# parlance/ctcdecode

Hardware: AMD Instinct MI355X
Metric: utterances/sec at B=256 T=1000 V=29 beam=100 (higher is better)
Workload: dtype f32; 1 GPU; BASELINE.json configs[1]: CTC prefix beam search, no LM, log-softmax of N(0,1) logits; HBM-resident tensors (input in HBM, the four result tensors left in HBM: `e2e`, with --full, is the host-to-host call); utterances_per_gpu=256, frames=1000, vocab=29, beam_width=100, cutoff_top_n=29, global_batch=256, ranks=1, devices_visible=1, parallelism=single GPU, threads_per_workgroup=default

## Files before the change

ctcdecode_amd/csrc/beam_core.h:

```cpp
#pragma once
#include <stddef.h>
#include <stdint.h>

#include "exact_math.h"
#include "exact_math_f64.h"
#include "lm_tables.h"
#include "stl_emul.h"
#if defined(CTC_ASSUME_CHECKED)
#include <cstdio>
#include <cstdlib>
#endif

#define CTC_RARE(x) __builtin_expect(!!(x), 0)
#if !defined(CTC_SPEC_UP)
#define CTC_SPEC_UP 1.5f
#endif
#if !defined(CTC_SPEC_DN)
#define CTC_SPEC_DN 0.7f
#endif
#if !defined(CTC_SPEC_OVER_SHIFT)
#define CTC_SPEC_OVER_SHIFT 2
#endif
#define CTC_USUAL(x) __builtin_expect(!!(x), 1)

namespace ctcbeam {

struct alignas(16) Int4v { int x, y, z, w; };

struct PoolNode {
  int32_t parent;
  float lpc;
  uint32_t cht;
  CTC_HD int ch() const { const uint32_t c = cht & 0xFFFFu; return c == 0xFFFFu ? -1 : (int)c; }
  CTC_HD static uint32_t pack(int ch, int tstep) { return ((uint32_t)ch & 0xFFFFu) | ((uint32_t)tstep << 16); }
};

struct EkWide { uint64_t k; uint32_t slot, pad; };
template <bool HUGE> struct EkOps;
template <> struct EkOps<false> {
  using E = uint64_t; using Pos = uint16_t;
  CTC_HD static E make(uint64_t key48v, int slot) { return (key48v << 16) | (uint64_t)slot; }
  CTC_HD static uint64_t key(const E &e) { return e >> 16; }
  CTC_HD static int slot(const E &e) { return (int)(e & 0xFFFFu); }
};
template <> struct EkOps<true> {
  using E = EkWide; using Pos = uint32_t;
  CTC_HD static E make(uint64_t key48v, int slot) { E e; e.k = key48v; e.slot = (uint32_t)slot; e.pad = 0; return e; }
  CTC_HD static uint64_t key(const E &e) { return e.k; }
  CTC_HD static int slot(const E &e) { return (int)e.slot; }
};

enum : uint32_t { T_SELF = 0, T_CHILD = 1, T_REVIVED = 2, T_HOLE = 3 };
enum : int { ST_OK = 0, ST_POOL_OVERFLOW = 1, ST_BAD_CONFIG = 2 };

constexpr int kMaxBeam = 16383;
constexpr int kMaxVocab = 65534;
constexpr int kIntMax = 0x7fffffff;

CTC_HD uint32_t ord_f32(float f) {
  const uint32_t u = ctcmath::f32_to_bits(f + 0.0f);
  return u ^ ((uint32_t)((int32_t)u >> 31) | 0x80000000u);
}
CTC_HD uint32_t ord_f32_raw(float f) {
  const uint32_t u = ctcmath::f32_to_bits(f);
  return u ^ ((uint32_t)((int32_t)u >> 31) | 0x80000000u);
}
CTC_HD float unord_f32(uint32_t k) {
  return ctcmath::bits_to_f32((k & 0x80000000u) ? (k ^ 0x80000000u) : ~k);
}
CTC_HD uint32_t mk_info(int ch, uint32_t type, int entry) {
  return ((uint32_t)(0xFFFF - (ch + 1)) << 16) | (type << 14) | (uint32_t)entry;
}
CTC_HD uint32_t info_type(uint32_t info) { return (info >> 14) & 3u; }
CTC_HD int info_entry(uint32_t info) { return (int)(info & 0x3FFFu); }
CTC_HD int info_ch(uint32_t info) { return 0xFFFF - (int)(info >> 16) - 1; }
CTC_HD uint64_t key48(uint32_t skey, uint32_t info) { return ((uint64_t)skey << 16) | (info >> 16); }
constexpr uint32_t kHoleInfo = T_HOLE << 14;

struct Beam {
  int *node, *par, *ch, *dep, *lcp, *via, *viaanc, *viach;
  int *up;
  float *bprev, *nbprev, *score, *lpc;
  int *lmst, *lmcl;
  int *acc_lo, *acc_hi;
  int *dn, *dmlo, *dmhi, *dfc;
  int *spc_lo, *spc_hi;
  int *spst, *spcl;
};
constexpr int kBeamArrays = 13, kBeamArraysLm = 12;

struct Dims {
  int K;
  int V;
  int Vc_max;
  int use_rank_table;
  int lm;
  CTC_HD int S_max() const { return K * (2 + Vc_max); }
};

enum {
  VAR_STATUS = 0, VAR_CUT, VAR_TAUC,
  VAR_INTO,
  VAR_FB0 = 4, VAR_FB1, VAR_FB2, VAR_FB3,
  VAR_TAU = 8, VAR_G, VAR_E,
  VAR_DANGER,
  VAR_PAR0 = 12,
  P_NPIN = 0, P_LCOUNT, P_NMAXKEY, P_NMINKEY, P_NCAND, P_SIZE = 8,
  VAR_SPEC = VAR_PAR0 + 2 * P_SIZE, SP_THR = 0, SP_WLOG, SP_ANCHOR, SP_PRED, SP_BEST, SP_MARGIN, SP_GAP, SP_ROWMAX,
  VAR_ROWMAX = VAR_SPEC + SP_ROWMAX,
  VAR_QSTAT = VAR_SPEC + 9,
  VAR_LMMISS = VAR_SPEC + 8,
  VAR_LMQ = VAR_SPEC + 10,
  VAR_HOTN = VAR_SPEC + 4,
  VAR_COUNT = VAR_SPEC + 12
};
constexpr int kBins = 1024;
constexpr int kBinsLog = 10;
constexpr int kListCap = 128;
constexpr int kSmallK = 128, kSmallV = 32;
constexpr int kMidK = 112, kMidVc = 40, kMidV = 10240;
constexpr int kWideK = 500, kWideV = 29;
CTC_HD constexpr Dims fixed_layout_dims(bool lm = false) { return Dims{kSmallK, kSmallV, kSmallV, 1, lm ? 1 : 0}; }
CTC_HD bool fits_fixed_layout(const Dims &d) { return d.K <= kSmallK && d.V <= kSmallV && d.Vc_max <= kSmallV; }
CTC_HD constexpr Dims mid_layout_dims() { return Dims{kMidK, kMidV, kMidVc, 1, 0}; }
CTC_HD bool fits_mid_layout(const Dims &d) { return d.K <= kMidK && d.V <= kMidV && d.Vc_max <= kMidVc && d.use_rank_table && !d.lm; }
CTC_HD constexpr Dims wide_layout_dims() { return Dims{kWideK, kWideV, kWideV, 0, 0}; }
CTC_HD bool fits_wide_layout(const Dims &d) { return d.K <= kWideK && d.V <= kWideV && d.Vc_max <= kWideV && !d.use_rank_table && !d.lm; }
constexpr int kHotCap = 256;
#if !defined(CTC_SERIAL_CUT)
#define CTC_SERIAL_CUT 12
#endif
constexpr int kSerialCut = CTC_SERIAL_CUT;
constexpr int kExpress = 32;
enum Event { EV_FRAMES, EV_CANDIDATES, EV_EXACT, EV_INTERNAL, EV_PINNED, EV_LPC_UPDATE, EV_DEAD_PARENT, EV_REVIVE_CAND, EV_REVIVED, EV_WALK,
             EV_WALK_HOPS, EV_FAST_SELECT, EV_SINGLE_KEY, EV_BUCKET_KEYS, EV_SPEC_OK, EV_SPEC_UNDER, EV_SPEC_OVER, EV_SPEC_OTHER, EV_SPEC_HOT,
             EV_SLOW_BELOW, EV_SLOW_CROWDED, EV_SLOW_SINGLE, EV_SLOW_ROUNDS, EV_TIE_FRAMES, EV_TIE_KEYS, EV_TIE_BIG, EV_WIDE_LIST, EV_HOT_LIST, EV_COUNT };

struct Work {
  Beam cur, nxt, beam0;
  size_t beam_blk;
  size_t beam_blk_far;
  size_t blk_via, blk_lm;
  int *e, *anc, *ostart, *cstart, *pinr, *revr;
  int *ancbuf, *acntbuf;
  uint32_t *hit;
  float *b_new, *nb_new, *sc_new, *rev_lpc;
  int *cch;
  float *clp;
  float *clpbuf;
  int16_t *rank_of;
  uint32_t *skey, *sinfo, *pos;
  int *surv;
  uint64_t *ek;
  uint16_t *lr;
  uint32_t *wpre;
  int *bins;
  int *hotge;
  int *lcpst;
  uint32_t *list;
  int *lslot;
  uint32_t *bitmap;
  int *fin, *sstack;
  int stage_skey;
  int *apos;
  int *vars;
};

template <class P>
CTC_HD P *carve_ptr(char *&p, size_t count) {
  P *r = reinterpret_cast<P *>(p);
  p += ((count * sizeof(P) + 15) / 16) * 16;
  return r;
}

template <int BIG, bool FARREP = false>
CTC_HD size_t carve(Work &w, char *base, char *far, const Dims &d, size_t *far_bytes) {
  char *p = base;
  char *q = far;
  constexpr bool deep = BIG >= 2;
  constexpr bool huge = BIG >= 3;
  const size_t K = (size_t)d.K, S = (size_t)d.S_max();
  const size_t Kr = ((K * 4 + 15) / 16) * 16;
  Beam *bs[2] = {&w.cur, &w.nxt};
  constexpr bool lm_far = BIG != 0;
  const size_t n_lm = d.lm ? (size_t)kBeamArraysLm : 0;
  w.beam_blk = (size_t)(kBeamArrays - (deep ? 3 : 0) + (lm_far ? 0 : n_lm)) * Kr;
  w.beam_blk_far = ((deep ? 3 : 0) + (lm_far ? n_lm : 0)) * Kr;
  w.blk_via = deep ? w.beam_blk_far : w.beam_blk;
  w.blk_lm = lm_far ? w.beam_blk_far : w.beam_blk;
  for (int i = 0; i < 2; ++i) {
    Beam &b = *bs[i];
    char *f = q + (size_t)i * w.beam_blk_far;
    b.node = carve_ptr<int>(p, K); b.par = carve_ptr<int>(p, K); b.ch = carve_ptr<int>(p, K);
    b.dep = carve_ptr<int>(p, K); b.lcp = carve_ptr<int>(p, K);
    char *&pv3 = deep ? f : p;
    b.via = carve_ptr<int>(pv3, K); b.viaanc = carve_ptr<int>(pv3, K); b.viach = carve_ptr<int>(pv3, K);
    b.up = carve_ptr<int>(p, K);
    b.bprev = carve_ptr<float>(p, K); b.nbprev = carve_ptr<float>(p, K); b.score = carve_ptr<float>(p, K);
    b.lpc = carve_ptr<float>(p, K);
    const size_t Kl = d.lm ? K : 0;
    char *&pl = lm_far ? f : p;
    b.lmst = carve_ptr<int>(pl, Kl); b.lmcl = carve_ptr<int>(pl, Kl); b.acc_lo = carve_ptr<int>(pl, Kl); b.acc_hi = carve_ptr<int>(pl, Kl);
    b.dn = carve_ptr<int>(pl, Kl); b.dmlo = carve_ptr<int>(pl, Kl); b.dmhi = carve_ptr<int>(pl, Kl); b.dfc = carve_ptr<int>(pl, Kl);
    b.spc_lo = carve_ptr<int>(pl, Kl); b.spc_hi = carve_ptr<int>(pl, Kl); b.spst = carve_ptr<int>(pl, Kl); b.spcl = carve_ptr<int>(pl, Kl);
  }
  q += 2 * w.beam_blk_far;
  w.beam0 = w.cur;
  w.e = carve_ptr<int>(p, K); w.ancbuf = carve_ptr<int>(p, 2 * K); w.acntbuf = carve_ptr<int>(p, 2 * K); w.anc = w.ancbuf;
  w.ostart = carve_ptr<int>(p, K);
  w.cstart = carve_ptr<int>(p, K);
  w.pinr = carve_ptr<int>(deep ? q : p, K);
  w.revr = carve_ptr<int>(deep ? q : p, K); w.hit = carve_ptr<uint32_t>(p, 2 * K);
  w.b_new = carve_ptr<float>(p, K); w.nb_new = carve_ptr<float>(p, K); w.sc_new = carve_ptr<float>(p, K);
  w.rev_lpc = carve_ptr<float>(deep ? q : p, K);
  w.cch = carve_ptr<int>(p, (size_t)d.Vc_max);
  w.clpbuf = carve_ptr<float>(p, 2 * (size_t)d.Vc_max); w.clp = w.clpbuf;
  w.rank_of = carve_ptr<int16_t>(p, d.use_rank_table ? (size_t)d.V : 0);
  w.skey = carve_ptr<uint32_t>(deep ? q : p, S);
  w.surv = carve_ptr<int>(p, 3 * K + 4);
  const size_t lcap = (d.K <= kSmallK && d.Vc_max <= kMidVc) ? (size_t)kHotCap + 64 : (size_t)kListCap + 4;
  w.bins = carve_ptr<int>(p, kBins + kBins / 16 + 4); w.list = carve_ptr<uint32_t>(p, lcap);
  w.lslot = carve_ptr<int>(p, lcap);
  w.hotge = carve_ptr<int>(p, lcap > (size_t)kListCap + 4 ? (size_t)kHotCap : 0);
#if defined(CTC_EXP_LCP_TABLE)
  w.lcpst = carve_ptr<int>(p, (lcap > (size_t)kListCap + 4 && !d.lm) ? (size_t)7 * kSmallK : 0);
#else
  w.lcpst = nullptr;
#endif
  w.bitmap = carve_ptr<uint32_t>(huge ? q : p, 2 * ((S + 63) / 64 + 17));
  w.wpre = huge ? carve_ptr<uint32_t>(q, (S + 63) / 64 + 2) : reinterpret_cast<uint32_t *>(w.bins);
  w.fin = carve_ptr<int>(BIG ? q : p, d.lm ? 2 * K : K);
  w.apos = carve_ptr<int>(BIG ? q : p, K);
  w.sstack = carve_ptr<int>(p, 3 * (2 * 32 + 2));
  w.vars = carve_ptr<int>(p, VAR_COUNT);
  w.sinfo = carve_ptr<uint32_t>(p, BIG ? K : S);
  w.pos = carve_ptr<uint32_t>(BIG ? q : p, K + 2);
  char *&rr = (BIG || FARREP) ? q : p;
  w.ek = carve_ptr<uint64_t>(rr, huge ? 2 * S : S); w.lr = carve_ptr<uint16_t>(rr, (2 * S + 2) * (huge ? 2 : 1));
  w.stage_skey = deep ? 0 : 1;
  if (far_bytes) *far_bytes = (size_t)(q - far);
  return (size_t)(p - base);
}

struct StreamState {
  int *hdr;
  int *arrays;
  int finish;
};
enum { SH_FRAMES = 0, SH_N, SH_POOL, SH_WLOG, SH_MAXKEY, SH_DANGER, SH_MINKEY,
       SH_SP_PRED, SH_SP_GAP, SH_SP_MARGIN,
       SH_WORDS = 12 };
constexpr int kStateArrays = 14;
constexpr int kStateArraysLm = kStateArrays + kBeamArraysLm;
CTC_HD int state_arrays(int lm) { return lm ? kStateArraysLm : kStateArrays; }

struct StepIn {
  int t;
  int Vc;
  int blank_rank;
  int identity;
  float blank_prob;
};


CTC_HD int div_p2(int v, int d) { return v >> __builtin_ctz((unsigned)d); }
CTC_HD int ceil_div_p2(int v, int d) { return div_p2(v + d - 1, d); }

CTC_HD double ctc_log_f64(double v) {
  return ctcmath::log_f64(v, ctcmath::tables64());
}

CTC_HD int ceil_log2_u32(uint32_t v) {
  return v <= 1u ? 0 : 32 - __builtin_clz(v - 1u);
}
CTC_HD int ceil_log2_u64(uint64_t v) {
  return v <= 1 ? 0 : 64 - __builtin_clzll(v - 1);
}

struct OutRefs {
  int32_t *tok, *ts;
  float *score;
  int32_t *len;
  int32_t *n_results;
  int K, T_stride;
  int32_t *c_hdr, *c_ent;
  uint32_t *c_rag;
  unsigned *c_count;
  unsigned c_cap;
  int32_t *m_hdr, *m_ent, *m_done;
  uint32_t *m_rag;
  unsigned m_cap;
};
enum : int { ST_COMPACT_OVERFLOW = 3, ST_INPUT_TIMEOUT = 4,
             ST_NEED_HOST = 5,
             ST_CB_DANGER = 6 };

struct SlotCtx {
  const Beam *pb;
  int n, Vnb, brank;
  uint64_t vmagic;
};

template <class X>
struct FullSyncView {
  X &x;
  CTC_HD int tid() const { return x.tid(); }
  CTC_HD int nt() const { return x.nt(); }
  CTC_HD void sync() { x.sync_full(); }
  CTC_HD int uni(int v) const { return x.uni(v); }
  CTC_HD void block_scan_u32(uint32_t mine, uint32_t *base_out, uint32_t *total_out) { x.block_scan_u32(mine, base_out, total_out); }
  CTC_HD int lanes() const { return x.lanes(); }
  CTC_HD auto ballot(bool p) const { return x.ballot(p); }
  template <class M> CTC_HD int count(M m) const { return x.count(m); }
  template <class M> CTC_HD int count_below(M m) const { return x.count_below(m); }
  CTC_HD uint32_t first_lane(uint32_t v) const { return x.first_lane(v); }
};

#if defined(CTC_ASSUME_CHECKED)
#define CTC_ASSUME(c) do { if (!(c)) { std::fprintf(stderr, "beam_core.h:%d: assumption violated: %s\n", __LINE__, #c); std::abort(); } } while (0)
#elif defined(__clang__)
#define CTC_ASSUME(c) __builtin_assume(c)
#else
#define CTC_ASSUME(c) do { if (!(c)) __builtin_unreachable(); } while (0)
#endif

template <class X, bool IDENT, int SMALLV = 0, bool LM = false, bool LAZY = false, bool FARREP = LAZY, bool HUGE = false, bool WORDLM = false, bool CB = false>
struct Decoder {
  using EO = EkOps<HUGE>;
  using Ek = typename EO::E;
  using LrT = typename EO::Pos;
  static constexpr int kClsK = SMALLV == 2 ? kMidK : kSmallK, kClsVc = SMALLV == 2 ? kMidVc : kSmallV, kClsSlots = kClsK * (2 + kClsVc);
  CTC_HD Ek *ekp() const { return reinterpret_cast<Ek *>(w.ek); }
  CTC_HD LrT *lrp() const { return reinterpret_cast<LrT *>(w.lr); }
  X &x;
  Work &w;
  const Dims d;
  const int blank;
  PoolNode *pool;
  int *pool_up;
  int *pool_thi;
  bool long_t = false;
  const int pool_cap;
  const uint64_t *tbl;
  const ctclm::LmView *lm;

  CTC_HD Decoder(X &x_, Work &w_, const Dims &d_, int blank_, PoolNode *pool_, int *pool_up_, int pool_cap_, const uint64_t *tbl_,
                 const ctclm::LmView *lm_ = nullptr)
      : x(x_), w(w_), d(d_), blank(blank_), pool(pool_), pool_up(pool_up_), pool_thi(pool_up_ + pool_cap_), pool_cap(pool_cap_), tbl(tbl_), lm(lm_) {
    if (LM) {
      const ctclm::DictNode root = lm->dict[0];
      root_lo = (int)root.mask_lo; root_hi = (int)root.mask_hi; root_fc = (int)root.first_child;
      lm_char_v = lm->char_based != 0; lm_wide_v = lm->dict_wide != 0; lm_space = lm->space_id;
      lm_alpha = lm->alpha; lm_beta = lm->beta;
      lm_dict = lm->dict;
    }
  }
  CTC_HD int node_tstep(const PoolNode &pn, int id) const { return (int)(pn.cht >> 16) | (CTC_RARE(long_t) ? pool_thi[id] << 16 : 0); }
  CTC_HD void set_node_time(int id, int ch, int tstep, float lpc) const {
    pool[id].lpc = lpc;
    pool[id].cht = PoolNode::pack(ch, tstep);
    if (CTC_RARE(long_t)) pool_thi[id] = tstep >> 16;
  }

  CTC_HD float lse(float a, float b) const { return ctcmath::lse(a, b, tbl); }

  static constexpr bool kRankEpoch = SMALLV == 2 && !IDENT && X::kRankEpoch;
  CTC_HD static int16_t rank_tag(int t, int r) { return (int16_t)(uint16_t)((((uint32_t)t & 1023u) << 6) | (uint32_t)r); }
  static constexpr bool kTailZero = IDENT && SMALLV && !LAZY && X::kZeroKeyTail;
  CTC_HD void zero_key_tail(int from) {
    if (!kTailZero) return;
    for (int i = from + x.tid(); i < kClsSlots; i += x.nt()) w.skey[i] = 0u;
  }

  static constexpr bool kSpec = SMALLV && (!LM || (X::kSpecLm && !CB)) && !LAZY && X::kSpecSelect;
#if defined(CTC_EXP_HOT_PRELIST)
  static constexpr bool kHotPre = LAZY && !LM && !SMALLV && !HUGE;
#else
  static constexpr bool kHotPre = false;
#endif
  struct HotPre { uint32_t thr; int cap; uint32_t *key; int *slot; };
  uint32_t st_gap = 0;
  uint32_t hot_anchor = 0;
  static constexpr bool kA1Overlap = kSpec && X::kA1Overlap;
  static constexpr bool kLcpTable = kSpec && X::kLcpTable;
  static constexpr bool kParentRec = !SMALLV && !LM && X::kParentRec && !kHotPre;
  static constexpr bool kLmOverlap = LM && WORDLM && SMALLV && !CB && !LAZY && X::kLmOverlap;
  static constexpr uint32_t kLmSpaceDeferred = 0x80000000u;
  CTC_HD void spec_learn(bool selected, uint32_t tau, int hot, int K) const {
    int *sp = w.vars + VAR_SPEC;
    const int pred = sp[SP_PRED];
    const float best = ctcmath::bits_to_f32((uint32_t)sp[SP_BEST]);
    float margin = ctcmath::bits_to_f32((uint32_t)sp[SP_MARGIN]);
    const uint32_t anchor = (uint32_t)sp[SP_ANCHOR];
    int wl = 32;
    float cut = 0.f;
    if (selected) {
      if (pred) {
        if (hot < K) margin = margin < 32.f ? margin * CTC_SPEC_UP : margin;
        else if (hot > K + (K >> CTC_SPEC_OVER_SHIFT) + 3) margin = margin > 0.001f ? margin * CTC_SPEC_DN : margin;
      }
      cut = (best - unord_f32(tau)) + margin;
      const uint32_t kgap = anchor > tau ? anchor - tau : 0u;
      wl = (kgap ? 32 - __builtin_clz(kgap) : 0) + 1;
      wl = wl < kBinsLog ? kBinsLog : (wl > 32 ? 32 : wl);
    }
    sp[SP_MARGIN] = (int)ctcmath::f32_to_bits(margin); sp[SP_GAP] = (int)ctcmath::f32_to_bits(cut);
    sp[SP_PRED] = selected ? 1 : 0; sp[SP_WLOG] = wl;
  }
  CTC_HD void spec_predict(int t) const {
    int *sp = w.vars + VAR_SPEC;
    const int pred = sp[SP_PRED];
    const float rowmax = ctcmath::bits_to_f32((uint32_t)sp[SP_ROWMAX]), cut = ctcmath::bits_to_f32((uint32_t)sp[SP_GAP]);
    const uint32_t mk = (uint32_t)pvars(t - 1)[P_NMAXKEY];
    const float best = unord_f32(mk) + rowmax;
    uint32_t k = ord_f32(best - cut);
    k = k ? k : 1u;
    k = pred ? k : 0xFFFFFFFFu;
    sp[SP_THR] = (int)k; sp[SP_BEST] = (int)ctcmath::f32_to_bits(best); sp[SP_ANCHOR] = (int)mk;
  }

  int st_n = 1, st_pool = 1, st_wlog = 32;
  uint32_t st_maxkey = 0;
  uint32_t st_minkey = 0;
  int root_lo = 0, root_hi = 0, root_fc = 0;
  bool lm_char_v = false, lm_wide_v = false;
  CTC_HD bool lm_char_() const { return !WORDLM && lm_char_v; }
  CTC_HD bool lm_wide_() const { return !WORDLM && lm_wide_v; }
  int lm_space = -1;
  double lm_alpha = 0.0, lm_beta = 0.0;
  const ctclm::DictNode *lm_dict = nullptr;
  static constexpr bool lm_cb = LM && CB;
  CTC_HD int *fin_cur() const { return w.fin + (lm_cb ? st_par * d.K : 0); }
  CTC_HD int *fin_nxt() const { return w.fin + (lm_cb ? (st_par ^ 1) * d.K : 0); }
  static constexpr int kLmqFilter = 256;
  CTC_HD static uint32_t *lmq_filter() {
#if defined(__HIP_DEVICE_COMPILE__)
    __shared__ uint32_t f[kLmqFilter];
#else
    static thread_local uint32_t f[kLmqFilter];
#endif
    return f;
  }
  CTC_HD void lmq_filter_clear() {
    if constexpr (lm_cb)
      for (int i = x.tid(); i < kLmqFilter; i += x.nt()) lmq_filter()[i] = 0u;
  }
  CTC_HD bool lmq_first(uint32_t state, uint32_t word) const {
    if constexpr (lm_cb) {
      if (lm->cb != 1) return true;
      const uint32_t h = ctclm::ng_hash(state, word);
      const uint32_t fp = ((state * 0x85EBCA77u) ^ (word * 0xC2B2AE3Du) ^ (h >> 8)) | 1u;
      uint32_t *e = lmq_filter() + (h & (kLmqFilter - 1));
      if (*e == fp) return false;
      *e = fp;
    }
    return true;
  }
  CTC_HD double lm_cond_(uint32_t *st, int *cl, uint32_t word, bool *missed = nullptr) const {
    const uint32_t st0 = *st;
    const int cl0 = *cl;
    const double v = ctclm::lm_cond(*lm, st, cl, word);
    if (CTC_RARE(lm_cb)) {
      if (v != v) {
        w.vars[VAR_LMMISS] = 1;
        if (lmq_first(st0, word)) {
          unsigned i = x.global_add(lm->cb_count, 1u);
          if (lm->cb_ring) i &= lm->cb_cap - 1;
          if (i < lm->cb_cap) lm->cb_miss[i] = ctclm::MissEntry{st0, word, (uint32_t)x.item(), 1u};
          x.atomic_add(&w.vars[VAR_LMQ], 1);
        }
// ... 542 lines not shown
      uint32_t *wl = reinterpret_cast<uint32_t *>(w.nxt.node);
      const int hot_n = kHotPre ? x.uni(w.vars[VAR_HOTN]) : 0;
      const bool from_hot = kHotPre && !wide && hp.thr != 0xFFFFFFFFu && hp.thr <= b32 && hot_n <= hp.cap;
      if (tid == 0 && from_hot) x.count(EV_HOT_LIST, 1);
      rank_bucket_ext(S, pv, b32, bspan, true, K - fb[1], fb[1], fb[3], wide ? wl : w.list, wide ? reinterpret_cast<int *>(wl + wcap + 4) : w.lslot,
                  from_hot ? &hp : nullptr, hot_n);
      return true;
    }
#else
    (void)hp;
    if (CTC_USUAL(fb[0] >= 0 && fb[3] <= kListCap && (wd.shift != 0 || fb[0] == kBins - 1))) {
      const uint32_t b32 = wd.lo + ((uint32_t)fb[0] << wd.shift);
      const uint32_t bspan = fb[0] == kBins - 1 ? 0xFFFFFFFFu - b32 : (1u << wd.shift) - 1u;
      if (tid == 0) { x.count(EV_FAST_SELECT, 1); x.count(EV_BUCKET_KEYS, fb[3]); if (fb[3] == 1) x.count(EV_SINGLE_KEY, 1); }
      if (kHotPre) {
        const int hot_n = x.uni(w.vars[VAR_HOTN]);
        const bool from_hot = hp.thr != 0xFFFFFFFFu && hp.thr <= b32 && hot_n <= hp.cap;
        if (tid == 0 && from_hot) x.count(EV_HOT_LIST, 1);
        rank_bucket_ext(S, pv, b32, bspan, true, K - fb[1], fb[1], fb[3], w.list, w.lslot, from_hot ? &hp : nullptr, hot_n);
      } else {
        rank_bucket(S, pv, b32, bspan, true, K - fb[1], fb[1], fb[3]);
      }
      return true;
    }
#endif
    uint64_t lo = wd.lo, hi = (uint64_t)1 << 32;
    int shift = wd.shift;
    int need = K, gbase = 0;
    bool first = true;
    for (;;) {
      const int bstar = fb[0], above = fb[1], total = fb[2], inb = fb[3];
      uint64_t blo = 0, bhi = 0;
      bool again = true;
      if (tid == 0) x.count(EV_SLOW_ROUNDS, 1);
      if (bstar < 0) {
        if (tid == 0) x.count(EV_SLOW_BELOW, 1);
        gbase += total; need -= total; hi = lo; lo = 1;
      } else {
        blo = lo + ((uint64_t)bstar << shift);
        bhi = (bstar == kBins - 1) ? hi : blo + ((uint64_t)1 << shift);
        if (bhi > hi) bhi = hi;
        if (shift == 0 && bstar < kBins - 1) {
          if (tid == 0) x.count(EV_SLOW_SINGLE, 1);
          if (tid == 0) { w.vars[VAR_TAU] = (int)(uint32_t)blo; w.vars[VAR_G] = gbase + above; w.vars[VAR_E] = inb; }
          x.sync();
          return false;
        }
        if (inb <= kListCap) again = false;
        else { if (tid == 0) x.count(EV_SLOW_CROWDED, 1); gbase += above; need -= above; lo = blo; hi = bhi; }
      }
      if (!again) {
        rank_bucket<true>(S, pv, (uint32_t)blo, (uint32_t)(bhi - blo - 1), first, need - above, gbase + above, inb);
        return first;
      }
      first = false;
      for (int i = tid; i < kBins; i += nt) w.bins[i] = 0;
      x.sync();
      const uint64_t width = hi - lo;
      shift = width <= (uint64_t)kBins ? 0 : ceil_log2_u64(width) - kBinsLog;
      const uint32_t lo32 = (uint32_t)lo, span = (uint32_t)(hi - lo - 1);
      for (int s0 = tid; s0 < S; s0 += 4 * nt) {
        uint32_t kk[4];
        for (int u = 0; u < 4; ++u) kk[u] = s0 + u * nt < S ? w.skey[s0 + u * nt] : 0u;
        for (int u = 0; u < 4; ++u) {
          const uint32_t k = kk[u], dk = k - lo32;
          if (k >= lo32 && dk <= span) {
            const uint32_t bk = dk >> shift;
            const int bb = bk < (uint32_t)(kBins - 1) ? (int)bk : kBins - 1;
            x.atomic_add(&w.bins[bb], 1);
          }
        }
      }
      x.sync();
      x.find_bucket(w.bins, need, &w.vars[VAR_FB0]);
      x.uni4(&w.vars[VAR_FB0], fb);
    }
  }

  CTC_HD bool resolve_by_character(int S, uint32_t tau, int m, int E, int *pv, const SlotCtx *lz = nullptr) {
    const int tid = x.tid(), nt = x.nt();
    if (E > kListCap) return false;
    if (tid == 0) { pv[P_LCOUNT] = 0; w.vars[VAR_CUT] = 0; }
    x.sync();
    for (int s = tid; s < S; s += nt)
      if (w.skey[s] == tau) w.list[x.atomic_add(&pv[P_LCOUNT], 1)] = ((LAZY ? info_of_slot(*lz, s) : w.sinfo[s]) >> 16) + 1u;
    x.sync();
    for (int q = tid; q < E; q += nt) {
      const uint32_t mine = w.list[q];
      int g = 0, e = 0;
      for (int r = 0; r < E; ++r) {
        const uint32_t o = w.list[r];
        g += o > mine;
        e += o == mine;
      }
      if (g < m && m <= g + e) { w.vars[VAR_TAUC] = (int)(mine - 1u); w.vars[VAR_CUT] = (g + e == m) ? 1 : 2; }
    }
    x.sync();
    return x.uni(w.vars[VAR_CUT]) == 1;
  }

  CTC_HD void build_lcp_table(const Beam &b, int n, int lane) const {
    int *st = w.lcpst;
    const int i0 = lane, i1 = lane + 64;
    int v0 = i0 < n ? b.lcp[i0] : kIntMax, v1 = i1 < n ? b.lcp[i1] : kIntMax;
    st[i0] = v0; st[i1] = v1;
    x.wave_lds_fence();
#if defined(__clang__)
#pragma unroll
#endif
    for (int l = 1; l <= 6; ++l) {
      const int h = 1 << (l - 1);
      const int *p = st + (l - 1) * kSmallK;
      const int a = p[i0 + h];
      const int c = i1 + h < kSmallK ? p[i1 + h] : kIntMax;
      v0 = a < v0 ? a : v0; v1 = c < v1 ? c : v1;
      st[l * kSmallK + i0] = v0; st[l * kSmallK + i1] = v1;
      x.wave_lds_fence();
    }
  }
  CTC_HD int lca_depth_tbl(int ja, int jb) const {
    const int lo = ja < jb ? ja : jb, hi = ja < jb ? jb : ja;
    const int len = hi - lo;
    const int l = 31 - __builtin_clz((unsigned)(len > 0 ? len : 1));
    const int *p = w.lcpst + l * kSmallK;
    const int same = w.cur.dep[ja];
    const int a = p[lo + 1 < kSmallK ? lo + 1 : kSmallK - 1], c = p[hi - (1 << l) + 1];
    const int m = a < c ? a : c;
    return len == 0 ? same : m;
  }
  CTC_HD int lca_depth(int ja, int jb) const {
    const Beam &b = w.cur;
    if (ja == jb) return b.dep[ja];
    const int lo = ja < jb ? ja : jb, hi = ja < jb ? jb : ja;
    int m = kIntMax;
    for (int i = lo + 1; i <= hi; i += 8) {
      const int i1 = i + 1 < hi ? i + 1 : hi, i2 = i + 2 < hi ? i + 2 : hi, i3 = i + 3 < hi ? i + 3 : hi;
      const int i4 = i + 4 < hi ? i + 4 : hi, i5 = i + 5 < hi ? i + 5 : hi, i6 = i + 6 < hi ? i + 6 : hi, i7 = i + 7 < hi ? i + 7 : hi;
      const int l0 = b.lcp[i], l1 = b.lcp[i1], l2 = b.lcp[i2], l3 = b.lcp[i3];
      const int l4 = b.lcp[i4], l5 = b.lcp[i5], l6 = b.lcp[i6], l7 = b.lcp[i7];
      const int m01 = l0 < l1 ? l0 : l1, m23 = l2 < l3 ? l2 : l3, m45 = l4 < l5 ? l4 : l5, m67 = l6 < l7 ? l6 : l7;
      const int ma = m01 < m23 ? m01 : m23, mb = m45 < m67 ? m45 : m67;
      const int mm = ma < mb ? ma : mb;
      m = mm < m ? mm : m;
    }
    return m;
  }

  template <class XX>
  CTC_HD int hoare_round(XX &xx, Ek *v, int first, int last, LrT *Lp, LrT *Rp) {
    if (FARREP) return stlemu::hoare_round_parallel<true>(xx, v, first, last, [](const Ek &e) { return EO::key(e); }, Lp, Rp, &w.vars[VAR_CUT]);
    return stlemu::hoare_round_parallel_chunks(xx, v, first, last, [](const Ek &e) { return EO::key(e); }, Lp, Rp, &w.vars[VAR_CUT]);
  }

  template <class XX>
  CTC_HD bool replay_nth_element(XX &fx, int N, int K) {
    const int tid = x.tid(), nt = x.nt();
    Ek *v = ekp();
    LrT *lr = lrp();
    auto before = [](const Ek &a, const Ek &c) { return EO::key(a) > EO::key(c); };
    int first = 0, last = N, depth = 2 * stlemu::floor_lg(N);
    if (!FARREP) {
      while (last - first > kSerialCut && depth > 0) {
        --depth;
        const int cut = hoare_round(x, v, first, last, lr, lr + N + 1);
        if (cut <= K) first = cut; else last = cut;
      }
      if (tid == 0) stlemu::introselect(v, first, K, last, depth, before);
      x.sync();
      return false;
    }
    Ek *sv = reinterpret_cast<Ek *>(w.nxt.node);
    int stage_cap = (int)((w.beam_blk - 16) / (sizeof(Ek) + 2 * sizeof(LrT)));
    if (w.stage_skey) {
      sv = reinterpret_cast<Ek *>(w.skey);
      const int cap_e = d.S_max() / 2, cap_p = (int)(w.beam_blk / 4) - 2;
      stage_cap = cap_e < cap_p ? cap_e : cap_p;
    }
    while (last - first > kSerialCut && depth > 0 && last - first > stage_cap) {
      --depth;
      const int cut = hoare_round(fx, v, first, last, lr, lr + N + 1);
      if (cut <= K) first = cut; else last = cut;
    }
    if (last - first > kSerialCut && depth > 0) {
      const int m0 = last - first, base = first;
      LrT *sLp = w.stage_skey ? reinterpret_cast<LrT *>(w.nxt.node) : reinterpret_cast<LrT *>(sv + m0), *sRp = sLp + m0 + 1;
      for (int i = tid; i < m0; i += nt) sv[i] = v[base + i];
      x.sync();
      int f2 = 0, l2 = m0;
      const int K2 = K - base;
      while (l2 - f2 > kSerialCut && depth > 0) {
        --depth;
        const int cut = hoare_round(x, sv, f2, l2, sLp, sRp);
        if (cut <= K2) f2 = cut; else l2 = cut;
      }
      if (tid == 0) stlemu::introselect(sv, f2, K2, l2, depth, before);
      x.sync();
      for (int i = tid; i < m0; i += nt) v[base + i] = sv[i];
      fx.sync();
      return w.stage_skey != 0;
    }
    if (tid == 0) stlemu::introselect(v, first, K, last, depth, before);
    fx.sync();
    return false;
  }

  CTC_HD void prime_a1(int t) {
    if (!kA1Overlap) return;
    select_beams();
    phase_a1(w.cur, st_n, w.ancbuf + (t & 1) * d.K, w.acntbuf + (t & 1) * d.K, x.group(), x.ngroups());
    x.sync();
  }
  CTC_HD void phase_a1(const Beam &b, int n, int *anc, int *acnt, int grp, int ngr) {
    const int rows = ceil_div_p2(n, ngr);
    auto entry_of = [=](int r) { return r * ngr + ((grp - r) & (ngr - 1)); };
    for (int k0 = 0; k0 < rows; k0 += x.lanes()) {
      const int k = k0 + x.lane();
      const int j = entry_of(k);
      bool internal = false;
      int dj = 0;
      if (k < rows && j < n) {
        dj = b.dep[j];
        internal = j + 1 < n && b.lcp[j + 1] >= dj;
        if (!internal) w.e[j] = j + 1;
      }
      unsigned long long todo = x.ballot(internal);
      if (internal) x.count(EV_INTERNAL, 1);
      if ((LM || (X::kQuarters && __builtin_popcountll(todo) >= 3)) && x.subtrees_by_quarters(todo, k0, grp, ngr, b.dep, b.lcp, n, w.e, anc, acnt)) todo = 0;
      while (todo) {
        const int kk = __builtin_ctzll(todo);
        todo &= todo - 1;
        const int jj = entry_of(k0 + kk);
        const int q = x.first_below(b.lcp, jj + 2, n, x.pick(dj, kk));
        if (x.lane() == 0) w.e[jj] = q;
        for (int c = jj + 1 + x.lane(); c < q; c += x.lanes()) {
          x.atomic_max(&anc[c], jj);
          x.atomic_add(&acnt[c], 1);
        }
      }
    }
  }

  CTC_HD int step(const StepIn &in, bool last, bool stage = false, float stage_val = 0.f, int next_cnt = 0, float next_val = 0.f) {
    select_beams();
    const Beam b = w.cur;
    const Beam nb = w.nxt;
    const int tid = x.tid_fresh(), nt = x.nt();
    const int n = st_n, pool_count = st_pool;
    const int K = d.K;
    const int Vc = in.Vc, brank = in.blank_rank;
    if (SMALLV) { CTC_ASSUME(n >= 1 && n <= kClsK); CTC_ASSUME(Vc >= 1 && Vc <= kClsVc); CTC_ASSUME(d.K <= kClsK); }
    const int Vnb = Vc - (brank >= 0 ? 1 : 0);
    const int S = n * (2 + Vnb);
    const bool small_vocab = SMALLV || Vnb <= 64;
    int *pv = pvars(in.t);
    int *surv = w.surv, *rk = w.surv + K, *ord = w.surv + 2 * K;
    Window wd{1u, 0};
    if (!kSpec) wd = first_window();
    HotPre hp{0xFFFFFFFFu, 0, nullptr, nullptr};
    if (kHotPre) {
      hp.cap = wide_list_cap();
      hp.key = reinterpret_cast<uint32_t *>(w.nxt.node);
      hp.slot = reinterpret_cast<int *>(hp.key + hp.cap + 4);
      if (x.tid() == 0) w.vars[VAR_HOTN] = 0;
    }
    float min_cutoff = CTC_NEG_MAX;
    bool full_beam = false;
    if (LM) {
      const double bpos = lm_beta > 0.0 ? lm_beta : 0.0;
      min_cutoff = (float)((double)(unord_f32(st_minkey) + in.blank_prob) - bpos);
      full_beam = n == K;
    }
    auto cut = [&](float lp, float prefix_score) { return LM && full_beam && lp + prefix_score < min_cutoff; };
    if (LM && CTC_RARE(x.uni(w.vars[VAR_DANGER]) != 0)) {
      lm_sorted_order(b, n);
    }

    w.anc = w.ancbuf + (in.t & 1) * K;
    int *acnt = w.acntbuf + (in.t & 1) * K;
    const bool lm_job = LM && !lm_char_();
    const int lm_joff = (SMALLV && x.nt_is(1024)) ? kSmallK : nt >= 2 * ((n + 63) & ~63) ? ((n + 63) & ~63) : 0;
    int lm_jk = -1;
    bool lm_defer = false;
    ctclm::DictNode lm_jinfo;
    if (lm_job) {
      const int k = tid - lm_joff;
      if (k >= 0 && k < n) {
        const int fc = b.dfc[k], dnk = b.dn[k];
        if (fc == kLmPending) {
          lm_jk = k; lm_jinfo = lm_dict[dnk];
          if (kLmOverlap) lm_defer = !(k + 1 < n && b.lcp[k + 1] >= b.dep[k]);
        }
      }
    }
    x.tick();
    if (!kA1Overlap) {
      phase_a1(b, n, w.anc, acnt, x.group(), x.ngroups());
      x.tick();
      x.sync();
    }
    if (kSpec && tid == x.spec_thread()) spec_predict(in.t);
    int npin = 0;
    Int4v *prec = reinterpret_cast<Int4v *>(w.nxt.node);
    for (int j = tid; j < n; j += nt) {
      const int dj = b.dep[j], q = w.e[j], P = w.anc[j], a = acnt[j];
      w.ostart[j] = 2 * j + Vnb * (j - a);
      const int cs_j = 2 * q + Vnb * (q - 1 - a);
      w.cstart[j] = cs_j;
      if (kParentRec) prec[j] = Int4v{(int)ctcmath::f32_to_bits(b.score[j]), (int)ctcmath::f32_to_bits(b.bprev[j]), cs_j, b.ch[j]};
      int pr = -1, rr = -1;
      if (P >= 0) {
        if (b.dep[P] == dj - 1) {
          pr = rank_of_char(in, b.ch[j]);
        } else {
          if (CTC_RARE(b.viaanc[j] != b.node[P])) {
            int hops = dj - b.dep[P] - 1, xn = b.node[j];
            x.count(EV_WALK, 1); x.count(EV_WALK_HOPS, hops);
#if !defined(CTC_NO_WALK_FROM_PARENT)
            int h0 = 0;
            if (LM && hops >= 1) { xn = b.par[j]; h0 = 1; }
            for (int h = h0; h < hops; ++h) xn = pool[xn].parent;
#else
            for (int h = 0; h < hops; ++h) xn = pool[xn].parent;
#endif
            b.via[j] = xn;
            b.viaanc[j] = b.node[P];
            b.viach[j] = pool[xn].ch();
          }
          if (b.lcp[j] <= b.dep[P]) rr = rank_of_char(in, b.viach[j]);
          x.count(EV_DEAD_PARENT, 1); if (rr >= 0) x.count(EV_REVIVE_CAND, 1);
        }
        const int r = pr >= 0 ? pr : rr;
        if (r >= 0 && small_vocab) {
          const int bit = r - ((brank >= 0 && r > brank) ? 1 : 0);
          x.atomic_or(&w.hit[hit_word(P, bit)], 1u << (bit & 31));
        }
      }
      w.pinr[j] = pr;
      w.revr[j] = rr;
      npin += pr >= 0;
    }
    if (x.group() * x.lanes() < n) {
      if (SMALLV && x.nt_is(1024)) x.wave_add_flag(&pv[P_NPIN], npin != 0);
      else x.wave_add(&pv[P_NPIN], npin);
    }
    const bool lm_ovl = kLmOverlap && lm_job;
    if (lm_job && tid >= lm_joff) {
      if (lm_jk >= 0) {
        if (lm_ovl && lm_defer) { b.dmlo[lm_jk] = (int)lm_jinfo.mask_lo; b.dmhi[lm_jk] = (int)kLmSpaceDeferred; b.dfc[lm_jk] = (int)lm_jinfo.first_child; }
        else lm_resolve_entry(b, lm_jk, lm_jinfo);
      }
      for (int k = tid - lm_joff + (nt - lm_joff); k < n; k += nt - lm_joff)
        if (b.dfc[k] == kLmPending) lm_resolve_entry(b, k, lm->dict[b.dn[k]]);
    }
    x.sync();
    x.mark(0);
// ... 1037 lines not shown
```

ctcdecode_amd/csrc/stl_emul.h:

```cpp
#pragma once
#include <stdint.h>

#if defined(__HIPCC__)
#define STLEMU_HD __host__ __device__ inline
#else
#define STLEMU_HD inline
#endif
#if defined(__HIP_DEVICE_COMPILE__)
#define STLEMU_FN __host__ __device__ __attribute__((noinline))
#else
#define STLEMU_FN STLEMU_HD
#endif

namespace stlemu {

STLEMU_HD int floor_lg(int n) {
  int k = 0;
  while (n > 1) {
    n >>= 1;
    ++k;
  }
  return k;
}

template <class T>
STLEMU_HD void exch(T *v, int a, int b) {
  T t = v[a];
  v[a] = v[b];
  v[b] = t;
}

template <class T, class C>
STLEMU_HD void median_to(T *v, int res, int a, int b, int c, C before) {
  if (before(v[a], v[b])) {
    if (before(v[b], v[c]))
      exch(v, res, b);
    else if (before(v[a], v[c]))
      exch(v, res, c);
    else
      exch(v, res, a);
  } else if (before(v[a], v[c])) {
    exch(v, res, a);
  } else if (before(v[b], v[c])) {
    exch(v, res, c);
  } else {
    exch(v, res, b);
  }
}

template <class T, class C>
STLEMU_HD int hoare_split(T *v, int lo, int hi, int piv, C before) {
  for (;;) {
    while (before(v[lo], v[piv])) ++lo;
    --hi;
    while (before(v[piv], v[hi])) --hi;
    if (!(lo < hi)) return lo;
    exch(v, lo, hi);
    ++lo;
  }
}

template <class T, class C>
STLEMU_FN int split_with_median_pivot(T *v, int first, int last, C before) {
  int mid = first + (last - first) / 2;
  median_to(v, first, first + 1, mid, last - 1, before);
  return hoare_split(v, first + 1, last, first, before);
}

template <class T, class C>
STLEMU_HD void sift(T *v, int base, int hole, int len, T value, C before) {
  const int top = hole;
  int child = hole;
  while (child < (len - 1) / 2) {
    child = 2 * (child + 1);
    if (before(v[base + child], v[base + child - 1])) --child;
    v[base + hole] = v[base + child];
    hole = child;
  }
  if ((len & 1) == 0 && child == (len - 2) / 2) {
    child = 2 * (child + 1);
    v[base + hole] = v[base + child - 1];
    hole = child - 1;
  }
  int parent = (hole - 1) / 2;
  while (hole > top && before(v[base + parent], value)) {
    v[base + hole] = v[base + parent];
    hole = parent;
    parent = (hole - 1) / 2;
  }
  v[base + hole] = value;
}

template <class T, class C>
STLEMU_HD void heapify(T *v, int first, int last, C before) {
  const int len = last - first;
  if (len < 2) return;
  int parent = (len - 2) / 2;
  for (;;) {
    T value = v[first + parent];
    sift(v, first, parent, len, value, before);
    if (parent == 0) return;
    --parent;
  }
}

template <class T, class C>
STLEMU_HD void pop_to(T *v, int first, int middle, int at, C before) {
  T value = v[at];
  v[at] = v[first];
  sift(v, first, 0, middle - first, value, before);
}

template <class T, class C>
STLEMU_FN void heap_select(T *v, int first, int middle, int last, C before) {
  heapify(v, first, middle, before);
  for (int i = middle; i < last; ++i)
    if (before(v[i], v[first])) pop_to(v, first, middle, i, before);
}

template <class T, class C>
STLEMU_FN void heap_sort_down(T *v, int first, int last, C before) {
  while (last - first > 1) {
    --last;
    pop_to(v, first, last, last, before);
  }
}

template <class T, class C>
STLEMU_FN void linear_insert_unguarded(T *v, int at, C before) {
  T value = v[at];
  int prev = at - 1;
  while (before(value, v[prev])) {
    v[at] = v[prev];
    at = prev;
    --prev;
  }
  v[at] = value;
}

template <class T, class C>
STLEMU_FN void insertion_sort(T *v, int first, int last, C before) {
  if (first == last) return;
  for (int i = first + 1; i != last; ++i) {
    if (before(v[i], v[first])) {
      T value = v[i];
      for (int j = i; j > first; --j) v[j] = v[j - 1];
      v[first] = value;
    } else {
      linear_insert_unguarded(v, i, before);
    }
  }
}

template <class T, class C>
STLEMU_HD void introselect(T *v, int first, int nth, int last, int depth, C before) {
  while (last - first > 3) {
    if (depth == 0) {
      heap_select(v, first, nth + 1, last, before);
      exch(v, first, nth);
      return;
    }
    --depth;
    int cut = split_with_median_pivot(v, first, last, before);
    if (cut <= nth)
      first = cut;
    else
      last = cut;
  }
  insertion_sort(v, first, last, before);
}

template <class T, class C>
STLEMU_HD void nth_element(T *v, int first, int nth, int last, C before) {
  if (first == last || nth == last) return;
  introselect(v, first, nth, last, 2 * floor_lg(last - first), before);
}

template <class T, class C>
STLEMU_HD void sort(T *v, int first, int last, C before, int *stack) {
  if (first == last) return;
  const int lo0 = first, hi0 = last;
  int sp = 0;
  int depth = 2 * floor_lg(last - first);
  for (;;) {
    while (last - first > 16) {
      if (depth == 0) {
        heap_select(v, first, last, last, before);
        heap_sort_down(v, first, last, before);
        break;
      }
      --depth;
      int cut = split_with_median_pivot(v, first, last, before);
      stack[sp++] = cut;
      stack[sp++] = last;
      stack[sp++] = depth;
      last = cut;
    }
    if (sp == 0) break;
    depth = stack[--sp];
    last = stack[--sp];
    first = stack[--sp];
  }
  first = lo0;
  last = hi0;
  if (last - first > 16) {
    insertion_sort(v, first, first + 16, before);
    for (int i = first + 16; i != last; ++i) linear_insert_unguarded(v, i, before);
  } else {
    insertion_sort(v, first, last, before);
  }
}

template <class X, class T, class C, class I>
STLEMU_HD void sort_parallel(X &x, T *v, int n, C before, I *cur, I *nxt, I *small, int *cnt, int seeded_tasks = -1,
                             int limit = 0x7fffffff) {
  const int tid = x.tid(), nt = x.nt();
  int ntask = seeded_tasks;
  if (seeded_tasks < 0) {
    if (tid == 0) {
      cnt[0] = 0; cnt[1] = 0; cnt[2] = 0;
      cur[0] = (I)0; cur[1] = (I)n; cur[2] = (I)(2 * floor_lg(n));
    }
    x.sync();
    ntask = 1;
  }
  for (int round = 0; ntask > 0; ++round) {
    int *c_next = cnt + (round & 1);
    for (int k = tid; k < ntask; k += nt) {
      const int first = (int)cur[3 * k], last = (int)cur[3 * k + 1], depth = (int)cur[3 * k + 2];
      if (depth == 0) {
        heap_select(v, first, last, last, before);
        heap_sort_down(v, first, last, before);
        continue;
      }
      const int cut = split_with_median_pivot(v, first, last, before);
      for (int side = 0; side < 2; ++side) {
        const int a = side ? cut : first, e = side ? last : cut;
        if (a >= limit) continue;
        if (e - a > 16) {
          const int i = x.atomic_add(c_next, 1);
          nxt[3 * i] = (I)a; nxt[3 * i + 1] = (I)e; nxt[3 * i + 2] = (I)(depth - 1);
        } else if (e - a > 1) {
          const int i = x.atomic_add(cnt + 2, 1);
          small[2 * i] = (I)a; small[2 * i + 1] = (I)e;
        }
      }
    }
    x.sync();
    ntask = x.uni(*c_next);
    if (tid == 0) cnt[(round + 1) & 1] = 0;
    I *t = cur; cur = nxt; nxt = t;
    x.sync();
  }
  const int nsmall = x.uni(cnt[2]);
  for (int k = tid; k < nsmall; k += nt) insertion_sort(v, (int)small[2 * k], (int)small[2 * k + 1], before);
  x.sync();
}

template <bool MEDIAN_BY_ALL = false, class X, class T, class KeyOf, class P>
STLEMU_HD int hoare_round_parallel(X &x, T *v, int first, int last, KeyOf key_of, P *Lp, P *Rp, int *cutvar) {
  const int tid = x.tid(), nt = x.nt();
  constexpr bool wide = sizeof(P) > 2;
  auto before = [&](const T &a, const T &b) { return key_of(a) > key_of(b); };
  const int lo = first + 1, m = last - lo;
  decltype(key_of(v[first])) kp;
  if (MEDIAN_BY_ALL) {
    const int pa = first + 1, pb = first + (last - first) / 2, pc = last - 1;
    const T va = v[pa], vb = v[pb], vc = v[pc], vf = v[first];
    int pm;
    if (before(va, vb)) pm = before(vb, vc) ? pb : (before(va, vc) ? pc : pa);
    else pm = before(va, vc) ? pa : (before(vb, vc) ? pc : pb);
    const T vm = pm == pa ? va : (pm == pb ? vb : vc);
    x.sync();
    if (tid == 0) { v[first] = vm; v[pm] = vf; }
    x.sync();
    kp = key_of(vm);
  } else {
    if (tid == 0) median_to(v, first, first + 1, first + (last - first) / 2, last - 1, before);
    x.sync();
    kp = key_of(v[first]);
  }
  const int W = x.lanes(), lane = tid % W, grp = tid / W, ng = nt / W;
  const int per = ((m + ng - 1) / ng + W - 1) / W * W;
  const int g0 = grp * per < m ? grp * per : m, g1 = g0 + per < m ? g0 + per : m;
  uint32_t mineL = 0, mineR = 0;
  for (int i = g0; i < g1; i += W) {
    const bool in = i + lane < g1;
    const auto k = in ? key_of(v[lo + i + lane]) : kp;
    mineL += (uint32_t)x.count(x.ballot(in && k <= kp));
    mineR += (uint32_t)x.count(x.ballot(in && k >= kp));
  }
  uint32_t runL, runR;
  int nL, nR;
  if (wide) {
    uint32_t totL, totR;
    x.block_scan_u32(lane == 0 ? mineL : 0u, &runL, &totL);
    x.block_scan_u32(lane == 0 ? mineR : 0u, &runR, &totR);
    nL = (int)totL; nR = (int)totR;
  } else {
    uint32_t run, tot;
    x.block_scan_u32(lane == 0 ? (mineL | (mineR << 16)) : 0u, &run, &tot);
    runL = run & 0xFFFFu; runR = run >> 16;
    nL = (int)(tot & 0xFFFFu); nR = (int)(tot >> 16);
  }
  runL = x.first_lane(runL); runR = x.first_lane(runR);
  for (int i = g0; i < g1; i += W) {
    const bool in = i + lane < g1;
    const auto k = in ? key_of(v[lo + i + lane]) : kp;
    const bool isL = in && k <= kp, isR = in && k >= kp;
    const auto bl = x.ballot(isL), br = x.ballot(isR);
    if (isL) Lp[runL + (uint32_t)x.count_below(bl)] = (P)(lo + i + lane);
    if (isR) Rp[nR - 1 - (int)(runR + (uint32_t)x.count_below(br))] = (P)(lo + i + lane);
    runL += (uint32_t)x.count(bl);
    runR += (uint32_t)x.count(br);
  }
  if (tid == 0) Rp[nR] = (P)first;
  x.sync();
  const int tmax = nL < nR + 1 ? nL : nR + 1;
  auto crossed = [&](int t) { return t >= nL || t > nR || Lp[t] >= Rp[t]; };
  for (int t = tid; t <= tmax; t += nt) {
    if (!crossed(t)) {
      exch(v, (int)Lp[t], (int)Rp[t]);
// ... 118 lines not shown
```

Before: 52100 utterances/s.

## Finish nth_element selection in wavefront registers instead of a single thread

Raises the cutoff at which the parallel Hoare partition rounds hand off to serial introselect, from 12 up to 64 elements for non-huge keys. The tail is finished by one wavefront holding one element per lane, using readlane and ballot masks to emulate the median-of-three partition and insertion sort, rather than by thread 0 working through memory. This is meant to cut block-wide parallel rounds and their syncs plus slow single-thread memory traffic. It adds readlane-heavy serial-like steps, a fallback path when depth runs out, and state packed into VAR_CUT.

```diff
diff --git a/ctcdecode_amd/csrc/beam_core.h b/ctcdecode_amd/csrc/beam_core.h
--- a/ctcdecode_amd/csrc/beam_core.h
+++ b/ctcdecode_amd/csrc/beam_core.h
@@ -131,6 +131,11 @@
 #define CTC_SERIAL_CUT 12
 #endif
 constexpr int kSerialCut = CTC_SERIAL_CUT;
+#if !defined(CTC_LANE_CUT)
+#define CTC_LANE_CUT 64
+#endif
+constexpr int kLaneCut = CTC_LANE_CUT;
+static_assert(kLaneCut >= 4 && kLaneCut <= 64, "one element per lane of a wavefront");
 constexpr int kExpress = 32;
 enum Event { EV_FRAMES, EV_CANDIDATES, EV_EXACT, EV_INTERNAL, EV_PINNED, EV_LPC_UPDATE, EV_DEAD_PARENT, EV_REVIVE_CAND, EV_REVIVED, EV_WALK,
              EV_WALK_HOPS, EV_FAST_SELECT, EV_SINGLE_KEY, EV_BUCKET_KEYS, EV_SPEC_OK, EV_SPEC_UNDER, EV_SPEC_OVER, EV_SPEC_OTHER, EV_SPEC_HOT,
@@ -316,6 +321,40 @@
   CTC_HD uint32_t first_lane(uint32_t v) const { return x.first_lane(v); }
 };
 
+struct LaneFinish { uint64_t e; int state; };
+#if defined(__HIP_DEVICE_COMPILE__)
+struct LaneArray {
+  uint64_t mine;
+  int n;
+  __device__ __forceinline__ static int lane() { return (int)__builtin_amdgcn_mbcnt_hi(~0u, __builtin_amdgcn_mbcnt_lo(~0u, 0u)); }
+  __device__ __forceinline__ uint64_t get(int i) const {
+    const uint32_t lo = (uint32_t)__builtin_amdgcn_readlane((int)(uint32_t)mine, i), hi = (uint32_t)__builtin_amdgcn_readlane((int)(uint32_t)(mine >> 32), i);
+    return ((uint64_t)hi << 32) | lo;
+  }
+  __device__ __forceinline__ void put(int i, uint64_t e) { if (lane() == i) mine = e; }
+  template <class F> __device__ __forceinline__ uint64_t mask(F pred) const { return __builtin_amdgcn_ballot_w64(lane() < n && pred(mine)); }
+};
+__device__ __forceinline__ LaneFinish replay_finish_in_lanes(uint64_t mine, int n_, int nth_, int depth_) {
+  const int n = __builtin_amdgcn_readfirstlane(n_), nth = __builtin_amdgcn_readfirstlane(nth_);
+  int depth = __builtin_amdgcn_readfirstlane(depth_), first = 0, last = n;
+  LaneArray a{mine, n};
+  const bool done = stlemu::introselect_indexed(a, first, nth, last, depth, [](uint64_t e) { return EkOps<false>::key(e); });
+  return LaneFinish{a.mine, first | (last << 8) | (depth << 16) | (done ? 0 : 1 << 24)};
+}
+#else
+struct ArrayAccess {
+  uint64_t *v;
+  int n;
+  uint64_t get(int i) const { return v[i]; }
+  void put(int i, uint64_t e) { v[i] = e; }
+  template <class F> uint64_t mask(F pred) const {
+    uint64_t m = 0;
+    for (int i = 0; i < n; ++i) m |= pred(v[i]) ? 1ull << i : 0ull;
+    return m;
+  }
+};
+#endif
+
 #if defined(CTC_ASSUME_CHECKED)
 #define CTC_ASSUME(c) do { if (!(c)) { std::fprintf(stderr, "beam_core.h:%d: assumption violated: %s\n", __LINE__, #c); std::abort(); } } while (0)
 #elif defined(__clang__)
@@ -1164,21 +1203,51 @@
     return stlemu::hoare_round_parallel_chunks(xx, v, first, last, [](const Ek &e) { return EO::key(e); }, Lp, Rp, &w.vars[VAR_CUT]);
   }
 
+  static constexpr int kCut = HUGE ? kSerialCut : kLaneCut;
+  template <class XX>
+  CTC_HD void finish_select(XX &sx, Ek *v, int first, int K, int last, int depth) {
+    const int tid = x.tid();
+    auto before = [](const Ek &a, const Ek &c) { return EO::key(a) > EO::key(c); };
+    if constexpr (!HUGE) {
+      if (CTC_USUAL(last - first <= kLaneCut)) {
+        const int n = last - first;
+#if defined(__HIP_DEVICE_COMPILE__)
+        if (tid < 64) {
+          const LaneFinish r = replay_finish_in_lanes(tid < n ? v[first + tid] : 0ull, n, K - first, depth);
+          if (tid < n) v[first + tid] = r.e;
+          if (tid == 0) w.vars[VAR_CUT] = r.state;
+        }
+#else
+        if (tid == 0) {
+          ArrayAccess a{v + first, n};
+          int f = 0, l = n, dleft = depth;
+          const bool done = stlemu::introselect_indexed(a, f, K - first, l, dleft, [](uint64_t e) { return EO::key(e); });
+          w.vars[VAR_CUT] = f | (l << 8) | (dleft << 16) | (done ? 0 : 1 << 24);
+        }
+#endif
+        sx.sync();
+        const int st = x.uni(w.vars[VAR_CUT]);
+        if (CTC_USUAL((st >> 24) == 0)) return;
+        last = first + ((st >> 8) & 255); depth = (st >> 16) & 255; first += st & 255;
+      }
+    }
+    if (tid == 0) stlemu::introselect(v, first, K, last, depth, before);
+    sx.sync();
+  }
+
   template <class XX>
   CTC_HD bool replay_nth_element(XX &fx, int N, int K) {
     const int tid = x.tid(), nt = x.nt();
     Ek *v = ekp();
     LrT *lr = lrp();
-    auto before = [](const Ek &a, const Ek &c) { return EO::key(a) > EO::key(c); };
     int first = 0, last = N, depth = 2 * stlemu::floor_lg(N);
     if (!FARREP) {
-      while (last - first > kSerialCut && depth > 0) {
+      while (last - first > kCut && depth > 0) {
         --depth;
         const int cut = hoare_round(x, v, first, last, lr, lr + N + 1);
         if (cut <= K) first = cut; else last = cut;
       }
-      if (tid == 0) stlemu::introselect(v, first, K, last, depth, before);
-      x.sync();
+      finish_select(x, v, first, K, last, depth);
       return false;
     }
     Ek *sv = reinterpret_cast<Ek *>(w.nxt.node);
@@ -1188,31 +1257,29 @@
       const int cap_e = d.S_max() / 2, cap_p = (int)(w.beam_blk / 4) - 2;
       stage_cap = cap_e < cap_p ? cap_e : cap_p;
     }
-    while (last - first > kSerialCut && depth > 0 && last - first > stage_cap) {
+    while (last - first > kCut && depth > 0 && last - first > stage_cap) {
       --depth;
       const int cut = hoare_round(fx, v, first, last, lr, lr + N + 1);
       if (cut <= K) first = cut; else last = cut;
     }
-    if (last - first > kSerialCut && depth > 0) {
+    if (last - first > kCut && depth > 0) {
       const int m0 = last - first, base = first;
       LrT *sLp = w.stage_skey ? reinterpret_cast<LrT *>(w.nxt.node) : reinterpret_cast<LrT *>(sv + m0), *sRp = sLp + m0 + 1;
       for (int i = tid; i < m0; i += nt) sv[i] = v[base + i];
       x.sync();
       int f2 = 0, l2 = m0;
       const int K2 = K - base;
-      while (l2 - f2 > kSerialCut && depth > 0) {
+      while (l2 - f2 > kCut && depth > 0) {
         --depth;
         const int cut = hoare_round(x, sv, f2, l2, sLp, sRp);
         if (cut <= K2) f2 = cut; else l2 = cut;
       }
-      if (tid == 0) stlemu::introselect(sv, f2, K2, l2, depth, before);
-      x.sync();
+      finish_select(x, sv, f2, K2, l2, depth);
       for (int i = tid; i < m0; i += nt) v[base + i] = sv[i];
       fx.sync();
       return w.stage_skey != 0;
     }
-    if (tid == 0) stlemu::introselect(v, first, K, last, depth, before);
-    fx.sync();
+    finish_select(fx, v, first, K, last, depth);
     return false;
   }
 
diff --git a/ctcdecode_amd/csrc/stl_emul.h b/ctcdecode_amd/csrc/stl_emul.h
--- a/ctcdecode_amd/csrc/stl_emul.h
+++ b/ctcdecode_amd/csrc/stl_emul.h
@@ -168,6 +168,53 @@
       last = cut;
   }
   insertion_sort(v, first, last, before);
+}
+
+template <class A, class KeyOf>
+STLEMU_HD bool introselect_indexed(A &a, int &first, int nth, int &last, int &depth, KeyOf key_of) {
+  while (last - first > 3) {
+    if (depth == 0) return false;
+    --depth;
+    const int pa = first + 1, pb = first + (last - first) / 2, pc = last - 1;
+    const auto va = a.get(pa), vb = a.get(pb), vc = a.get(pc), vf = a.get(first);
+    const auto ka = key_of(va), kb = key_of(vb), kc = key_of(vc);
+    int pm;
+    if (ka > kb) pm = kb > kc ? pb : (ka > kc ? pc : pa);
+    else pm = ka > kc ? pa : (kb > kc ? pc : pb);
+    const auto vm = pm == pa ? va : (pm == pb ? vb : vc);
+    a.put(first, vm);
+    a.put(pm, vf);
+    const auto kp = key_of(vm);
+    int lo = first + 1, hi = last;
+    for (;;) {
+      const uint64_t le = a.mask([&](decltype(vm) e) { return key_of(e) <= kp; });
+      const uint64_t ge = a.mask([&](decltype(vm) e) { return key_of(e) >= kp; });
+      lo += __builtin_ctzll(le >> lo);
+      --hi;
+      hi = 63 - __builtin_clzll(ge & (~0ull >> (63 - hi)));
+      if (!(lo < hi)) break;
+      const auto tl = a.get(lo), th = a.get(hi);
+      a.put(lo, th);
+      a.put(hi, tl);
+      ++lo;
+    }
+    if (lo <= nth) first = lo; else last = lo;
+  }
+  for (int i = first + 1; i < last; ++i) {
+    const auto value = a.get(i);
+    if (key_of(value) > key_of(a.get(first))) {
+      for (int j = i; j > first; --j) a.put(j, a.get(j - 1));
+      a.put(first, value);
+    } else {
+      int at = i;
+      while (key_of(value) > key_of(a.get(at - 1))) {
+        a.put(at, a.get(at - 1));
+        --at;
+      }
+      a.put(at, value);
+    }
+  }
+  return true;
 }
 
 template <class T, class C>
```

After: 52770 utterances/s (median of 6 runs). +1.3%, better.
